# Mictronics/multi-sdr-gps-sim

Hardware: NVIDIA H100
Metric: IQ Msamples/s (higher is better)
Workload: dtype f64 NCO / int32 accumulate / int8 out

## Files before the change

include/gpsb200.h:

```cpp
#ifndef GPSB200_H
#define GPSB200_H

#include <stdbool.h>
#include <stddef.h>
#include <stdint.h>

#ifdef __cplusplus
extern "C" {
#endif

#define GPSB200_SAMPLERATE        3000000
#define GPSB200_BLOCK_SAMPLES     300000
#define GPSB200_BLOCK_ELEMS       600000
#define GPSB200_MAX_CHAN          32
#define GPSB200_NAV_WORDS         60
#define GPSB200_CA_LEN            1023
#define GPSB200_SC08              1
#define GPSB200_SC16              2
#define GPSB200_HACKRF_BUFFER     262144

enum {
    GPSB200_OK = 0,
    GPSB200_ERR_ARG = -1,
    GPSB200_ERR_CUDA = -2,
// ... 55 lines not shown

int gpsb200_synth_blocks_device(gpsb200_ctx_t *ctx, const gpsb200_chan_t *chans, int nblk, int nchan,
                                int sample_size, void *dst_device, void *stream,
                                double *carr_phase_out, gpsb200_stats_t *stats);

typedef struct gpsb200_slice_link {
    int32_t prn_first[GPSB200_MAX_CHAN];
    int32_t prn_last[GPSB200_MAX_CHAN];
    int32_t reset_inside[GPSB200_MAX_CHAN];
    double first_phase[GPSB200_MAX_CHAN];
    double value[GPSB200_MAX_CHAN];
} gpsb200_slice_link_t;
int gpsb200_slice_prepare(gpsb200_ctx_t *ctx, const gpsb200_chan_t *chans, int nblk, int nchan, int sample_size,
                          void *dst_device, void *dst_host, void *stream, gpsb200_slice_link_t *link);
int gpsb200_slice_wait(gpsb200_ctx_t *ctx);
int gpsb200_slice_probe(gpsb200_ctx_t *ctx, const int32_t *prn_in, const double *phase_guess_in, int eager);
int gpsb200_slice_finish(gpsb200_ctx_t *ctx, const int32_t *prn_in, const double *phase_in, int32_t *prn_out,
                         double *phase_out, gpsb200_stats_t *stats);
typedef void (*gpsb200_handoff_fn)(void *user, const int32_t *prn_out, const double *phase_out);
int gpsb200_slice_finish_cb(gpsb200_ctx_t *ctx, const int32_t *prn_in, const double *phase_in, int32_t *prn_out,
                            double *phase_out, gpsb200_stats_t *stats, gpsb200_handoff_fn handoff, void *user);
int gpsb200_slice_link_host(const gpsb200_chan_t *chans, int nblk, int nchan, gpsb200_slice_link_t *link);
int gpsb200_link_apply(const gpsb200_slice_link_t *link, int nchan, const int32_t *prn_in, const double *phase_in,
                       int32_t *prn_out, double *phase_out);

int gpsb200_debug_corrupt_chain(gpsb200_ctx_t *ctx, int on);

int gpsb200_debug_run_checkpoints(gpsb200_ctx_t *ctx, int nblk, int nchan, void *out);

int gpsb200_debug_block_probes(gpsb200_ctx_t *ctx, int nblk, int nchan, void *probes_out, double *seg_out,
                               double *guess_out);

int gpsb200_debug_synth_shape(gpsb200_ctx_t *ctx, int nblk, int nchan, int sample_size, const char **kernel,
                              int *ctas_per_block, int *runs_per_cta);

const char *gpsb200_synth_kernel_name(const gpsb200_ctx_t *ctx, int nchan);

int gpsb200_replay_device(gpsb200_ctx_t *ctx, void *dst_device, void *stream, int kernel_mask);

double gpsb200_carrier_advance(double carr_phase, double f_carr, int64_t nsamples);

int gpsb200_carrier_chain(const gpsb200_chan_t *chans, int nblk, int nchan, const double *phase_in,
                          double *phase_out, int threads);

int gpsb200_carrier_chain_device(gpsb200_ctx_t *ctx, const gpsb200_chan_t *chans, int nblk, int nchan,
                                 const double *phase_in, double *phase_out);

int gpsb200_carrier_probe_fixup(double start, double guess, double f_carr, int64_t nsamples, double *end_out);

int gpsb200_span_chain_host(const double *f_carr, int nblk, double start_true, double start_guess, double *starts_out);

int gpsb200_checkpoint_segments_host(double start_true, double start_guess, double f_carr, int run_samples,
                                     double *starts_out, int *nseg_out);

int gpsb200_carrier_probe_host(double guess, double f_carr, int64_t nsamples, int run_samples, int mode, void *probe_out,
                               double *seg_out);

int gpsb200_lanes_model_block(const gpsb200_chan_t *chans, int nchan, const uint32_t *nav, int run_samples, int force,
                              int16_t *iq, double *carr_out, int64_t *counters, uint32_t *signs);

int gpsb200_lanes_window_band_host(const uint32_t *steps, const uint32_t *bases, int64_t n, uint8_t *out);

int gpsb200_codegen(int prn, uint8_t ca[GPSB200_CA_LEN]);

#define GPSB200_ACQ_MAX_MS    100
#define GPSB200_ACQ_MAX_BINS  1024
#define GPSB200_ACQ_CODE_SAMPLES 3000
typedef struct gpsb200_acq_config {
    int64_t s0;
    int32_t ms;
    int32_t nprn;
    int32_t prn[32];
    double f_lo_hz;
    double step_hz;
    int32_t nbins;
    int32_t reserved;
} gpsb200_acq_config_t;
typedef struct gpsb200_acq_result {
    int32_t prn;
    int32_t bin;
    int32_t delay;
    int32_t reserved;
    double doppler_hz;
    double delay_chips;
    uint64_t p1, p2;
    double ratio;
} gpsb200_acq_result_t;
int gpsb200_acquire(gpsb200_ctx_t *ctx, const void *iq, int64_t nsamples, int sample_size, const gpsb200_acq_config_t *cfg,
                    gpsb200_acq_result_t *res, uint64_t *grid);
int gpsb200_acquire_device(gpsb200_ctx_t *ctx, const void *iq_device, int64_t nsamples, int sample_size,
                           const gpsb200_acq_config_t *cfg, gpsb200_acq_result_t *res, uint64_t *grid, void *stream);
int gpsb200_acquire_windows(gpsb200_ctx_t *ctx, const void *iq, int64_t nsamples, int sample_size,
                            const gpsb200_acq_config_t *cfg, const double *f_lo_prn, gpsb200_acq_result_t *res,
                            uint64_t *grid);
int gpsb200_debug_acq_split(gpsb200_ctx_t *ctx, int force, int nprn, int nbins);
int gpsb200_acquire_windows_device(gpsb200_ctx_t *ctx, const void *iq_device, int64_t nsamples, int sample_size,
                                   const gpsb200_acq_config_t *cfg, const double *f_lo_prn, gpsb200_acq_result_t *res,
                                   uint64_t *grid, void *stream);

#define GPSB200_TRK_CODE_STEP_NOM 1464583848u
#define GPSB200_TRK_CODE_STEP_MIN 1464095816u
#define GPSB200_TRK_CODE_STEP_MAX 1465072205u
#define GPSB200_TRK_FLL_EPOCHS    200
#define GPSB200_TRK_MAX_CHAN      32
typedef struct gpsb200_track_state {
    int32_t prn;
// ... 383 lines not shown
```

multi-sdr-gps-sim_b200/__init__.py:

```python
from .api import (
    BLOCK_ELEMS, BLOCK_SAMPLES, SC08, SC16, Chan, Config, Context, GpsB200Error, Stats,
    bind_numa, carrier_advance, span_chain_host, lanes_model_block, lanes_window_band, link_apply, slice_link_host, SliceLink, carrier_chain, codegen, scenario, lib, lib_path, CHAN_DTYPE,
    ScenarioConfig, LiveScenario, SteerState, parse_steer, KEYS, ERR_END, almanac_read, ALMANAC_RECORD_DTYPE, checkpoint_segments_host, RUN_CKPT_DTYPE,
    carrier_probe_host, CARRIER_PROBE_DTYPE, AcqConfig, ACQ_RESULT_DTYPE, ACQ_CODE_SAMPLES, acq_window_samples,
    TRACK_STATE_DTYPE, TRACK_EPOCH_DTYPE, NAV_BIT_DTYPE, NAV_WORD_DTYPE, NAV_SYNC_DTYPE, track_start, nav_decode, nav_word_check,
    nav_parity, EPHEMERIS_DTYPE, IONO_DTYPE, PVT_CHAN_DTYPE, PVT_CONFIG_DTYPE, FIX_DTYPE, FIX_OK, FIX_FEW,
    FIX_NO_CONVERGENCE, PVT_MAX_ITER, nav_words_of_frame, nav_ephemeris, nav_time_anchor, pvt_config,
    RAIM_CONFIG_DTYPE, RAIM_DTYPE, RAIM_PASS, RAIM_EXCLUDED, RAIM_ALERT, RAIM_UNAVAILABLE, RAIM_MAX_DOF,
    RAIM_MAX_EXCLUDE, raim_config, raim_thresholds, ARAIM_CONFIG_DTYPE, ARAIM_DTYPE, araim_config, araim_kfa,
    COARSE_CONFIG_DTYPE, COARSE_DTYPE, FIX_AMBIGUOUS, coarse_config, rinex_ephemeris,
    SEARCH_CONFIG_DTYPE, SEARCH_DTYPE, SEARCH_NODES, search_config, search_nodes,
    SKY_DTYPE, nav_almanac, almanac_predict,
    SNAPSHOT_CONFIG_DTYPE, SNAPSHOT_DTYPE, SNAP_OK, SNAP_WEAK, SNAP_NO_CONVERGENCE, SNAP_ITERATIONS, SNAP_MAX_ITER,
    snapshot_config,
)
from .synthetic import synthetic_chans
from . import sharding
```

multi-sdr-gps-sim_b200/api.py:

```python
import ctypes as C
import os

import numpy as np

BLOCK_SAMPLES = 300000
BLOCK_ELEMS = 600000
SC08, SC16 = 1, 2

_HERE = os.path.dirname(os.path.abspath(__file__))


def lib_path():
    return os.path.join(_HERE, "libgpsb200.so")


class GpsB200Error(RuntimeError):
    def __init__(self, code, msg):
        super().__init__("gpsb200 error %d: %s" % (code, msg))
        self.code = code


class Chan(C.Structure):
    _fields_ = [("prn", C.c_int32), ("iword", C.c_int32), ("ibit", C.c_int32), ("icode", C.c_int32),
                ("nav_frame", C.c_int32), ("reserved", C.c_int32),
# ... 292 lines not shown
    return rec, int(wna.value)


SKY_DTYPE = np.dtype([("prn", "<i4"), ("valid", "<i4"), ("el_deg", "<f8"), ("az_deg", "<f8"), ("range_m", "<f8"),
                      ("doppler_hz", "<f8")])
assert SKY_DTYPE.itemsize == 40


def almanac_predict(rec, week, sow, x_a):
    r = np.ascontiguousarray(rec, dtype=ALMANAC_RECORD_DTYPE)
    assert r.size == 32
    x = np.ascontiguousarray(x_a, dtype=np.float64).reshape(3)
    out = np.zeros(32, SKY_DTYPE)
    rc = lib().gpsb200_almanac_predict(r.ctypes.data, int(week), float(sow), x.ctypes.data, out.ctypes.data)
    if rc:
        raise GpsB200Error(rc, "gpsb200_almanac_predict")
    return out


def nav_time_anchor(words, sync):
    w = np.ascontiguousarray(words, dtype=NAV_WORD_DTYPE)
    sy = np.array(sync, dtype=NAV_SYNC_DTYPE).reshape(1)
    ep, ms = C.c_int32(0), C.c_int64(0)
    rc = lib().gpsb200_nav_time_anchor(w.ctypes.data if w.size else None, w.size, sy.ctypes.data, C.byref(ep), C.byref(ms))
    if rc:
        raise GpsB200Error(rc, "gpsb200_nav_time_anchor")
    return int(ep.value), int(ms.value)


def pvt_config(s0, step, nfix, iono=None):
    c = np.zeros(1, PVT_CONFIG_DTYPE)[0]
    c["s0"], c["step"], c["nfix"] = int(s0), int(step), int(nfix)
    if iono is not None:
        c["iono"] = 1
        c["alpha"], c["beta"] = np.asarray(iono[0], np.float64), np.asarray(iono[1], np.float64)
    return c


HANDOFF_FN = C.CFUNCTYPE(None, C.c_void_p, C.POINTER(C.c_int32), C.POINTER(C.c_double))

_lib = None

EXPORTS = ["gpsb200_create", "gpsb200_destroy", "gpsb200_last_error", "gpsb200_version", "gpsb200_set_nav",
           "gpsb200_synth_blocks", "gpsb200_synth_blocks_scatter", "gpsb200_synth_blocks_device", "gpsb200_replay_device",
           "gpsb200_carrier_advance", "gpsb200_carrier_chain", "gpsb200_carrier_chain_device", "gpsb200_carrier_probe_fixup",
           "gpsb200_codegen", "gpsb200_acquire", "gpsb200_acquire_device", "gpsb200_acquire_windows",
           "gpsb200_acquire_windows_device", "gpsb200_debug_acq_split", "gpsb200_nav_almanac", "gpsb200_almanac_predict", "gpsb200_track_start",
           "gpsb200_track",
           "gpsb200_track_device", "gpsb200_nav_decode", "gpsb200_nav_word_check", "gpsb200_nav_parity",
           "gpsb200_nav_ephemeris", "gpsb200_nav_time_anchor", "gpsb200_pvt", "gpsb200_pvt_replay",
           "gpsb200_pvt_raim", "gpsb200_raim_thresholds", "gpsb200_pvt_araim", "gpsb200_araim_kfa", "gpsb200_pvt_coarse", "gpsb200_pvt_search", "gpsb200_search_nodes", "gpsb200_snapshot_measure", "gpsb200_snapshot_measure_device", "gpsb200_pvt_snapshot", "gpsb200_pvt_snapshot_search", "gpsb200_rinex_ephemeris", "gpsb200_bind_numa", "gpsb200_span_chain_host", "gpsb200_lanes_model_block",
           "gpsb200_lanes_window_band_host", "gpsb200_slice_prepare", "gpsb200_slice_probe",
           "gpsb200_slice_finish", "gpsb200_slice_finish_cb", "gpsb200_slice_wait", "gpsb200_link_apply", "gpsb200_slice_link_host", "gpsb200_debug_corrupt_chain", "gpsb200_synth_kernel_name",
           "gpsb200_debug_run_checkpoints", "gpsb200_checkpoint_segments_host",
           "gpsb200_carrier_probe_host", "gpsb200_debug_block_probes", "gpsb200_debug_synth_shape",
           "gpsb200_scenario_create", "gpsb200_scenario_destroy", "gpsb200_scenario_error",
           "gpsb200_scenario_blocks", "gpsb200_scenario_channels", "gpsb200_scenario_nav_frames",
           "gpsb200_scenario_chans", "gpsb200_scenario_nav", "gpsb200_scenario_almanac_date", "gpsb200_almanac_read",
           "gpsb200_scenario_open", "gpsb200_scenario_advance", "gpsb200_scenario_frame", "gpsb200_scenario_key",
           "gpsb200_scenario_steer_state", "gpsb200_scenario_open_now", "gpsb200_scenario_create_now",
           "gpsb200_scenario_start_date", "gpsb200_scenario_start_time",
           "fifo_create", "fifo_destroy", "fifo_wait_next", "fifo_wait_full", "fifo_halt", "fifo_acquire",
           "fifo_enqueue", "fifo_dequeue", "fifo_release", "fifo_set_compat_drop",
           "gpsb200_iqfile_start", "gpsb200_iqfile_stop", "gpsb200_fifo_push", "gpsb200_fifo_push_flush"]


def lib():
    global _lib
    if _lib is None:
        if not os.path.exists(lib_path()):
            raise GpsB200Error(-2, "libgpsb200.so not built (run __graft_entry__.build()); there is no CPU fallback")
        L = C.CDLL(lib_path())
        L.gpsb200_create.argtypes = [C.POINTER(Config), C.POINTER(C.c_void_p)]
        L.gpsb200_destroy.argtypes = [C.c_void_p]
        L.gpsb200_last_error.argtypes = [C.c_void_p]
        L.gpsb200_last_error.restype = C.c_char_p
        L.gpsb200_version.restype = C.c_char_p
        L.gpsb200_set_nav.argtypes = [C.c_void_p, C.c_int, C.c_int, C.c_void_p]
        L.gpsb200_synth_blocks.argtypes = [C.c_void_p, C.c_void_p, C.c_int, C.c_int, C.c_int, C.c_void_p,
                                           C.c_void_p, C.POINTER(Stats)]
        L.gpsb200_synth_blocks_scatter.argtypes = [C.c_void_p, C.c_void_p, C.c_int, C.c_int, C.c_int, C.c_void_p,
                                                   C.c_void_p, C.POINTER(Stats)]
        L.gpsb200_synth_blocks_device.argtypes = [C.c_void_p, C.c_void_p, C.c_int, C.c_int, C.c_int, C.c_void_p,
                                                  C.c_void_p, C.c_void_p, C.POINTER(Stats)]
        L.gpsb200_replay_device.argtypes = [C.c_void_p, C.c_void_p, C.c_void_p, C.c_int]
        L.gpsb200_carrier_advance.argtypes = [C.c_double, C.c_double, C.c_int64]
        L.gpsb200_carrier_advance.restype = C.c_double
        L.gpsb200_codegen.argtypes = [C.c_int, C.c_void_p]
        L.gpsb200_scenario_create.argtypes = [C.POINTER(ScenarioConfig), C.POINTER(C.c_void_p)]
        L.gpsb200_scenario_destroy.argtypes = [C.c_void_p]
        L.gpsb200_scenario_error.argtypes = [C.c_void_p]
        L.gpsb200_scenario_error.restype = C.c_char_p
        for fn in ("blocks", "channels", "nav_frames"):
            getattr(L, "gpsb200_scenario_" + fn).argtypes = [C.c_void_p]
        L.gpsb200_scenario_chans.argtypes = [C.c_void_p]
        L.gpsb200_scenario_chans.restype = C.c_void_p
        L.gpsb200_scenario_nav.argtypes = [C.c_void_p]
        L.gpsb200_scenario_nav.restype = C.c_void_p
        L.gpsb200_scenario_almanac_date.argtypes = [C.c_void_p]
        L.gpsb200_scenario_almanac_date.restype = C.c_char_p
        L.gpsb200_almanac_read.argtypes = [C.c_char_p, C.c_void_p, C.POINTER(C.c_int32)]
        L.gpsb200_scenario_open.argtypes = [C.POINTER(ScenarioConfig), C.POINTER(C.c_void_p)]
        L.gpsb200_scenario_open_now.argtypes = [C.POINTER(ScenarioConfig), C.POINTER(C.c_void_p)]
        L.gpsb200_scenario_create_now.argtypes = [C.POINTER(ScenarioConfig), C.POINTER(C.c_void_p)]
        L.gpsb200_scenario_start_date.argtypes = [C.c_void_p]
        L.gpsb200_scenario_start_date.restype = C.c_char_p
        L.gpsb200_scenario_start_time.argtypes = [C.c_void_p, C.POINTER(C.c_int32), C.POINTER(C.c_double)]
        L.gpsb200_scenario_advance.argtypes = [C.c_void_p, C.c_int, C.c_void_p, C.POINTER(C.c_int32)]
        L.gpsb200_scenario_frame.argtypes = [C.c_void_p, C.c_int]
        L.gpsb200_scenario_frame.restype = C.c_void_p
        L.gpsb200_scenario_key.argtypes = [C.c_void_p, C.c_int]
        L.gpsb200_scenario_steer_state.argtypes = [C.c_void_p, C.POINTER(SteerState)]
        L.gpsb200_carrier_probe_fixup.argtypes = [C.c_double, C.c_double, C.c_double, C.c_int64, C.POINTER(C.c_double)]
        L.gpsb200_carrier_chain_device.argtypes = [C.c_void_p, C.c_void_p, C.c_int, C.c_int, C.c_void_p, C.c_void_p]
        L.gpsb200_carrier_chain.argtypes = [C.c_void_p, C.c_int, C.c_int, C.c_void_p, C.c_void_p, C.c_int]
        L.gpsb200_span_chain_host.argtypes = [C.c_void_p, C.c_int, C.c_double, C.c_double, C.c_void_p]
        L.gpsb200_slice_prepare.argtypes = [C.c_void_p, C.c_void_p, C.c_int, C.c_int, C.c_int, C.c_void_p, C.c_void_p,
                                            C.c_void_p, C.POINTER(SliceLink)]
        L.gpsb200_slice_finish_cb.argtypes = [C.c_void_p, C.c_void_p, C.c_void_p, C.c_void_p, C.c_void_p, C.POINTER(Stats),
                                              HANDOFF_FN, C.c_void_p]
        L.gpsb200_slice_wait.argtypes = [C.c_void_p]
        L.gpsb200_slice_link_host.argtypes = [C.c_void_p, C.c_int, C.c_int, C.POINTER(SliceLink)]
        L.gpsb200_slice_probe.argtypes = [C.c_void_p, C.c_void_p, C.c_void_p, C.c_int]
        L.gpsb200_slice_finish.argtypes = [C.c_void_p, C.c_void_p, C.c_void_p, C.c_void_p, C.c_void_p, C.POINTER(Stats)]
        L.gpsb200_link_apply.argtypes = [C.POINTER(SliceLink), C.c_int, C.c_void_p, C.c_void_p, C.c_void_p, C.c_void_p]
        L.gpsb200_debug_corrupt_chain.argtypes = [C.c_void_p, C.c_int]
        L.gpsb200_debug_run_checkpoints.argtypes = [C.c_void_p, C.c_int, C.c_int, C.c_void_p]
        L.gpsb200_checkpoint_segments_host.argtypes = [C.c_double, C.c_double, C.c_double, C.c_int, C.c_void_p,
                                                       C.POINTER(C.c_int)]
        L.gpsb200_carrier_probe_host.argtypes = [C.c_double, C.c_double, C.c_int64, C.c_int, C.c_int, C.c_void_p,
                                                 C.c_void_p]
        L.gpsb200_debug_block_probes.argtypes = [C.c_void_p, C.c_int, C.c_int, C.c_void_p, C.c_void_p, C.c_void_p]
        L.gpsb200_debug_synth_shape.argtypes = [C.c_void_p, C.c_int, C.c_int, C.c_int, C.POINTER(C.c_char_p),
                                                C.POINTER(C.c_int), C.POINTER(C.c_int)]
        L.gpsb200_synth_kernel_name.argtypes = [C.c_void_p, C.c_int]
        L.gpsb200_synth_kernel_name.restype = C.c_char_p
        L.gpsb200_acquire.argtypes = [C.c_void_p, C.c_void_p, C.c_int64, C.c_int, C.POINTER(AcqConfig), C.c_void_p,
                                      C.c_void_p]
        L.gpsb200_acquire_device.argtypes = [C.c_void_p, C.c_void_p, C.c_int64, C.c_int, C.POINTER(AcqConfig),
                                             C.c_void_p, C.c_void_p, C.c_void_p]
        L.gpsb200_acquire_windows.argtypes = [C.c_void_p, C.c_void_p, C.c_int64, C.c_int, C.POINTER(AcqConfig),
                                              C.c_void_p, C.c_void_p, C.c_void_p]
        L.gpsb200_acquire_windows_device.argtypes = [C.c_void_p, C.c_void_p, C.c_int64, C.c_int, C.POINTER(AcqConfig),
                                                     C.c_void_p, C.c_void_p, C.c_void_p, C.c_void_p]
        L.gpsb200_debug_acq_split.argtypes = [C.c_void_p, C.c_int, C.c_int, C.c_int]
        L.gpsb200_nav_almanac.argtypes = [C.c_void_p, C.c_int64, C.c_int32, C.c_void_p, C.POINTER(C.c_int32)]
        L.gpsb200_almanac_predict.argtypes = [C.c_void_p, C.c_int32, C.c_double, C.c_void_p, C.c_void_p]
        L.gpsb200_track_start.argtypes = [C.c_int, C.c_double, C.c_int64, C.c_void_p]
        L.gpsb200_track.argtypes = [C.c_void_p, C.c_void_p, C.c_int64, C.c_int, C.c_int64, C.c_void_p, C.c_int, C.c_int,
                                    C.c_void_p, C.c_void_p]
        L.gpsb200_track_device.argtypes = [C.c_void_p, C.c_void_p, C.c_int64, C.c_int, C.c_int64, C.c_void_p, C.c_int,
                                           C.c_int, C.c_void_p, C.c_void_p, C.c_void_p]
        L.gpsb200_nav_decode.argtypes = [C.c_void_p, C.c_int64, C.c_void_p, C.c_int64, C.c_void_p, C.c_int64, C.c_void_p]
        L.gpsb200_nav_word_check.argtypes = [C.c_uint32, C.c_uint32, C.POINTER(C.c_uint32)]
        L.gpsb200_nav_parity.argtypes = [C.c_uint32, C.c_int, C.c_int]
        L.gpsb200_nav_parity.restype = C.c_uint32
        L.gpsb200_nav_ephemeris.argtypes = [C.c_void_p, C.c_int64, C.c_void_p, C.c_void_p]
        L.gpsb200_nav_time_anchor.argtypes = [C.c_void_p, C.c_int64, C.c_void_p, C.POINTER(C.c_int32),
                                              C.POINTER(C.c_int64)]
        L.gpsb200_pvt.argtypes = [C.c_void_p, C.c_void_p, C.c_int, C.c_void_p, C.c_void_p, C.c_int, C.c_void_p, C.c_void_p,
                                  C.c_void_p]
        L.gpsb200_pvt_replay.argtypes = [C.c_void_p, C.c_void_p]
        L.gpsb200_pvt_raim.argtypes = [C.c_void_p, C.c_void_p, C.c_int, C.c_void_p, C.c_void_p, C.c_int, C.c_void_p,
                                       C.c_void_p, C.c_void_p, C.c_void_p, C.c_void_p]
        L.gpsb200_raim_thresholds.argtypes = [C.c_double, C.c_double, C.c_void_p, C.c_void_p]
        L.gpsb200_pvt_araim.argtypes = L.gpsb200_pvt_raim.argtypes
        L.gpsb200_araim_kfa.argtypes = [C.c_double, C.c_double, C.c_void_p, C.c_void_p]
        L.gpsb200_pvt_coarse.argtypes = L.gpsb200_pvt_raim.argtypes + [C.c_void_p]
        L.gpsb200_pvt_search.argtypes = L.gpsb200_pvt_coarse.argtypes + [C.c_void_p]
        L.gpsb200_search_nodes.argtypes = [C.c_int, C.c_void_p]
        L.gpsb200_snapshot_measure.argtypes = [C.c_void_p, C.c_void_p, C.c_int64, C.c_int, C.POINTER(AcqConfig),
                                               C.c_void_p, C.c_void_p, C.c_void_p]
        L.gpsb200_snapshot_measure_device.argtypes = L.gpsb200_snapshot_measure.argtypes + [C.c_void_p]
        L.gpsb200_pvt_snapshot.argtypes = [C.c_void_p, C.c_void_p, C.c_int, C.c_void_p, C.c_void_p, C.c_void_p,
                                           C.c_void_p, C.c_void_p, C.c_void_p, C.c_void_p]
        L.gpsb200_pvt_snapshot_search.argtypes = L.gpsb200_pvt_snapshot.argtypes + [C.c_void_p]
        L.gpsb200_rinex_ephemeris.argtypes = [C.c_char_p, C.c_int, C.c_int32, C.c_double, C.c_void_p]
        _lib = L
    return _lib


def bind_numa(device=0):
# ... 26 lines not shown
        raise GpsB200Error(rc, "gpsb200_carrier_chain")
    return out


def lanes_model_block(chans_row, nav_frame, run_samples=2400, force=0, want_signs=False):
    a = np.ascontiguousarray(chans_row, dtype=CHAN_DTYPE)
    nv = np.ascontiguousarray(nav_frame, dtype=np.uint32)
    iq = np.zeros(BLOCK_ELEMS, np.int16)
    co = np.zeros(a.size, np.float64)
    cnt = np.zeros(4, np.int64)
    signs = np.zeros((a.size, BLOCK_SAMPLES // 96, 3), np.uint32) if want_signs else None
    L = lib()
    L.gpsb200_lanes_model_block.argtypes = [C.c_void_p, C.c_int, C.c_void_p, C.c_int, C.c_int, C.c_void_p, C.c_void_p, C.c_void_p,
                                            C.c_void_p]
    rc = L.gpsb200_lanes_model_block(a.ctypes.data, a.size, nv.ctypes.data, run_samples, force, iq.ctypes.data, co.ctypes.data,
                                     cnt.ctypes.data, None if signs is None else signs.ctypes.data)
    if rc:
        raise GpsB200Error(rc, "gpsb200_lanes_model_block")
    return (iq, co, cnt, signs) if want_signs else (iq, co, cnt)


def lanes_window_band(steps, bases):
    st, bs = np.broadcast_arrays(np.asarray(steps, np.uint32), np.asarray(bases, np.uint32))
    st = np.ascontiguousarray(st.ravel())
    bs = np.ascontiguousarray(bs.ravel())
    out = np.zeros(st.size, np.uint8)
    L = lib()
    L.gpsb200_lanes_window_band_host.argtypes = [C.c_void_p, C.c_void_p, C.c_int64, C.c_void_p]
    rc = L.gpsb200_lanes_window_band_host(st.ctypes.data, bs.ctypes.data, st.size, out.ctypes.data)
    if rc:
        raise GpsB200Error(rc, "gpsb200_lanes_window_band_host")
    return out.astype(bool)


def span_chain_host(f_carr, start_true, start_guess):
    f = np.ascontiguousarray(f_carr, dtype=np.float64)
    out = np.zeros(f.size + 1)
    rc = lib().gpsb200_span_chain_host(f.ctypes.data, f.size, float(start_true), float(start_guess), out.ctypes.data)
    if rc < 0:
        raise GpsB200Error(rc, "gpsb200_span_chain_host")
    return out if rc == 1 else None


def checkpoint_segments_host(start_true, start_guess, f_carr, run_samples=2400):
    out = np.zeros(8)
    nseg = C.c_int(0)
    rc = lib().gpsb200_checkpoint_segments_host(float(start_true), float(start_guess), float(f_carr), int(run_samples),
                                            out.ctypes.data, C.byref(nseg))
    if rc < 0:
        raise GpsB200Error(rc, "gpsb200_checkpoint_segments_host")
    return rc == 1, out[:nseg.value]


def carrier_probe_host(guess, f_carr, nsamples=BLOCK_SAMPLES, run_samples=2400, mode=1):
    probe = np.zeros(1, CARRIER_PROBE_DTYPE)
    seg = np.zeros((2, 7))
    rc = lib().gpsb200_carrier_probe_host(float(guess), float(f_carr), int(nsamples), int(run_samples), int(mode),
                                          probe.ctypes.data, seg.ctypes.data)
    if rc:
        raise GpsB200Error(rc, "gpsb200_carrier_probe_host")
    return probe[0], seg


def slice_link_host(chans):
    a = np.ascontiguousarray(chans, dtype=CHAN_DTYPE)
    link = SliceLink()
    rc = lib().gpsb200_slice_link_host(a.ctypes.data, a.shape[0], a.shape[1], C.byref(link))
    if rc:
        raise GpsB200Error(rc, "gpsb200_slice_link_host")
    return link


def link_apply(link, nchan, prn_in=None, phase_in=None):
    pi = None if prn_in is None else np.ascontiguousarray(prn_in, dtype=np.int32)
    xi = None if phase_in is None else np.ascontiguousarray(phase_in, dtype=np.float64)
    po, xo = np.zeros(nchan, np.int32), np.zeros(nchan, np.float64)
    rc = lib().gpsb200_link_apply(C.byref(link), nchan, None if pi is None else pi.ctypes.data,
                                  None if xi is None else xi.ctypes.data, po.ctypes.data, xo.ctypes.data)
    if rc:
        raise GpsB200Error(rc, "gpsb200_link_apply")
    return po, xo


def almanac_read(path):
    rec = np.zeros(32, ALMANAC_RECORD_DTYPE)
    valid = C.c_int32(0)
    rc = lib().gpsb200_almanac_read(os.fsencode(path), rec.ctypes.data, C.byref(valid))
    if rc:
        raise GpsB200Error(rc, "cannot open almanac file %s" % path)
    return bool(valid.value), rec


def _scenario_config(nav_file, lat, lon, height, seconds, max_chan=12, motion_file=None, start=None,
                     ionosphere=True, pluto_gain=False, rinex3=False, target=None, almanac_file=None, interactive=False):
    cfg = ScenarioConfig()
    cfg.nav_file = os.fsencode(nav_file)
    cfg.motion_file = os.fsencode(motion_file) if motion_file else None
    cfg.lat_deg, cfg.lon_deg, cfg.height_m = lat, lon, height
    cfg.duration_ds = int(seconds * 10.0 + 0.5)
    cfg.max_chan = max_chan
    cfg.ionosphere_enable = 1 if ionosphere else 0
    cfg.pluto_gain = 1 if pluto_gain else 0
    cfg.rinex3 = 1 if rinex3 else 0
    cfg.almanac_file = os.fsencode(almanac_file) if almanac_file else None
    cfg.interactive = 1 if interactive else 0
    if target is not None:
# ... 478 lines not shown
```

multi-sdr-gps-sim_b200/csrc/gpsb200_api.cu:

```cuda
#include <cuda_runtime.h>
#include <sched.h>

#include <algorithm>
#include <atomic>
#include <chrono>
#include <condition_variable>
#include <functional>
#include <mutex>
#include <cctype>
#include <cmath>
#include <cstdio>
#include <cstring>
#include <memory>
#include <string>
#include <thread>
#include <vector>

#include "../../include/gpsb200.h"
#include "acquire.h"
#include "snapshot.h"
#include "device_buffer.h"
#include "track.h"
#include "pvt.h"
#include "nco_exact.h"
// ... 665 lines not shown
    CU(cudaEventRecord(ctx->ev[kEvCallEnd], call.stream));
    CU(cudaMemcpyAsync(ctx->h_chain_errors, ctx->d_chain_errors, sizeof(int), cudaMemcpyDeviceToHost, sp));
    ctx->last = call_args(ctx, call, 0, call.nblk);
    ctx->have_last = true;
    return GPSB200_OK;
}

int call_verdict(gpsb200_ctx *ctx, const Call &call) {
    int bad = *ctx->h_chain_errors;
    for (int i = 0; i < call.rows; i++)
        for (int c = 0; c < call.nchan; c++) {
            const double want = ctx->seg_expect[(size_t) i * call.nchan + c];
            if (want >= 0.0 && f64_bits(want) != f64_bits(ctx->h_seg_end[(size_t) i * call.nchan + c])) ++bad;
        }
    if (bad != 0)
        return fail(ctx, GPSB200_ERR_INTERNAL, "carrier chain self-check failed on " + std::to_string(bad) + " blocks");
    return GPSB200_OK;
}

void seed_chain(std::vector<ChainState> &chain, int nchan, const int32_t *prn_in, const double *phase_in) {
    for (int c = 0; c < nchan; c++) {
        chain[c].prn = (prn_in && phase_in && prn_in[c] > 0) ? prn_in[c] : 0;
        chain[c].phase = chain[c].prn ? phase_in[c] : 0.0;
    }
}

void export_chain(const std::vector<ChainState> &chain, int nchan, int32_t *prn_out, double *phase_out) {
    for (int c = 0; c < nchan; c++) {
        if (prn_out) prn_out[c] = chain[c].prn;
        if (phase_out) phase_out[c] = chain[c].prn > 0 ? chain[c].phase : 0.0;
    }
}

int small_call(gpsb200_ctx *ctx, Call &call, double *carr_phase_out, gpsb200_stats_t *stats) {
    const int nblk = call.nblk, nchan = call.nchan;
    cudaStream_t s = call.stream;
    double t0 = now_ms();
    int rc = prepare_blocks(ctx, call.chans, 0, nblk, nchan, call.chain);
    if (rc) return rc;
    const int nruns = ctx->nruns, run = ctx->cfg.run_samples;
    ctx->pool->run(nchan, [&](int c_lo, int c_hi) {
        for (int c = c_lo; c < c_hi; c++) {
            ChainState stc = call.chain[c];
            for (int b = 0; b < nblk; b++) {
                const BlockChanDev &p = ctx->h_bc[(size_t) b * nchan + c];
                RunCkpt *ck = ctx->h_ck + (size_t) b * nruns * nchan + c;
                if (p.prn <= 0) {
                    stc.prn = 0;
                    for (int r = 0; r < nruns; r++) ck[(size_t) r * nchan] = RunCkpt{0.0, 0.0, 0u, 0u};
                    continue;
                }
                if (stc.prn != p.prn) stc.phase = p.carr_in;
                stc.prn = p.prn;
                double x = stc.phase, y = p.code0;
                int iword = p.nav0 & 0xFF, ibit = (p.nav0 >> 8) & 0xFF, icode = (p.nav0 >> 16) & 0xFF;
                const WalkConst wx = walk_const(p.c_carr), wy = walk_const(p.c_code);
                for (int r = 0; r < nruns; r++) {
                    ck[(size_t) r * nchan] = RunCkpt{x, y, (uint32_t) iword | ((uint32_t) ibit << 8) | ((uint32_t) icode << 16), 0u};
                    int64_t periods = 0, dummy = 0;
                    nco_advance<NCO_CARRIER>(x, wx, run, dummy);
                    nco_advance<NCO_CODE>(y, wy, run, periods);
                    nav_advance(iword, ibit, icode, periods);
                }
                stc.phase = x;
            }
            call.chain[c] = stc;
        }
    });
    call.st.host_chain_ms = now_ms() - t0;
    rc = upload_nav(ctx, s);
    if (rc) return rc;
    const size_t cnt = (size_t) nblk * nchan;
    CU(cudaEventRecord(ctx->ev[kEvCallStart], s));
    CU(cudaMemcpyAsync(ctx->d_bc, ctx->h_bc, cnt * sizeof(BlockChanDev), cudaMemcpyHostToDevice, s));
    CU(cudaMemcpyAsync(ctx->d_ck, ctx->h_ck, cnt * nruns * sizeof(RunCkpt), cudaMemcpyHostToDevice, s));
    const SynthArgs a = call_args(ctx, call, 0, nblk);
    CU(launch_tables(a, s));
    CU(launch_synth(a, s));
    CU(cudaEventRecord(ctx->ev[kEvCallEnd], s));
    call.st.launches = 2;
    call.st.h2d_bytes = (int64_t) (cnt * (sizeof(BlockChanDev) + nruns * sizeof(RunCkpt)));
    if (call.host()) {
        rc = download(ctx, call, 0, nblk, s);
        if (rc) return rc;
        CU(cudaStreamSynchronize(s));
    }
    ctx->have_last = false;
    export_chain(call.chain, nchan, nullptr, carr_phase_out);
    if (stats) *stats = call.st;
    return GPSB200_OK;
}

int run_pipeline(gpsb200_ctx *ctx, Call &call, double *carr_phase_out, gpsb200_stats_t *stats) {
    ctx->trace_t0 = now_ms();
    trace(ctx, "call");
    if (call.nblk <= kHostChainBlocks && !ctx->fault_inject_chain) return small_call(ctx, call, carr_phase_out, stats);
    cudaStream_t sp = ctx->s_pre;
    int rc = call_open(ctx, call);
    if (rc) return rc;
    const auto &segs = call.segs;
    const int nseg = (int) segs.size();
    if (!call.host()) {
        std::vector<ChainState> guess = call.chain;
        for (int i = 0; i < nseg; i++) {
            cudaStream_t sw = (i & 1) ? ctx->s_ck : sp;
            rc = seg_params(ctx, call, segs[i].first, segs[i].second, sw, &guess, nullptr);
            if (rc) return rc;
            rc = seg_probe(ctx, call, segs[i].first, segs[i].second, sw);
            if (rc) return rc;
            CU(cudaEventRecord(ctx->ev_seg[i], sw));
        }
        trace(ctx, "speculative work enqueued");
        for (int i = 0; i < nseg; i++) {
            rc = seg_scan(ctx, call, i, ctx->ev_seg[i], nullptr);
            if (rc) return rc;
        }
        CU(cudaStreamSynchronize(ctx->s_ck));
// ... 291 lines not shown
const char *gpsb200_last_error(const gpsb200_ctx_t *ctx) { return ctx ? ctx->err.c_str() : "null context"; }

int gpsb200_codegen(int prn, uint8_t ca[GPSB200_CA_LEN]) { return ca_code(prn, ca) == 0 ? GPSB200_OK : GPSB200_ERR_ARG; }

double gpsb200_carrier_advance(double carr_phase, double f_carr, int64_t nsamples) {
    const double c = f_carr * (1.0 / (double) GPSB200_SAMPLERATE);
    int64_t dummy = 0;
    nco_advance<NCO_CARRIER>(carr_phase, c, nsamples, dummy);
    return carr_phase;
}

int gpsb200_carrier_probe_fixup(double start, double guess, double f_carr, int64_t nsamples, double *end_out) {
    const double c = f_carr * (1.0 / (double) GPSB200_SAMPLERATE);
    CarrierProbe p;
    carrier_probe(guess, c, nsamples, p);
    double xe = 0.0;
    const bool ok = carrier_fixup(start, c, p, xe);
    if (ok && end_out) *end_out = xe;
    return ok ? 1 : 0;
}

int gpsb200_span_chain_host(const double *f_carr, int nblk, double start_true, double start_guess, double *starts_out) {
    if (!f_carr || nblk < 1 || !starts_out) return GPSB200_ERR_ARG;
    const double delt = 1.0 / (double) GPSB200_SAMPLERATE;
    std::vector<CarrierProbe> probes(nblk);
    std::vector<double> cc(nblk);
    std::vector<SpanBlockState> spec(nblk);
    uint64_t acc = phase_to_fix(start_guess);
    const double guess0 = fix_to_phase(acc);
    for (int j = 0; j < nblk; j++) {
        cc[j] = f_carr[j] * delt;
        carrier_probe(fix_to_phase(acc), cc[j], GPSB200_BLOCK_SAMPLES, probes[j]);
        acc = guess_block(acc, cc[j]);
    }
    CarrierProbe sum{}, part{};
    bool ok[2];
    for (int V = 0; V < 2; V++) {
        span_chain(probes.data(), OneSatellite{cc.data()}, nblk, 1, guess0, V, part, ok[V], spec.data());
        if (V == 0) {
            sum.x_w = part.x_w;
            sum.n_w = part.n_w;
        }
        sum.x_end[V] = part.x_end[V];
        sum.m_pos[V] = ok[V] ? part.m_pos[V] : 0.0;
        sum.m_neg[V] = ok[V] ? part.m_neg[V] : 0.0;
    }
    double xe, d;
    int v;
    if (!carrier_fixup(start_true, cc[0], sum, xe, &v, &d, 1.0)) return 0;
    starts_out[0] = start_true;
    for (int j = 1; j < nblk; j++) starts_out[j] = spec[j].start[v] + d;
    starts_out[nblk] = xe;
    return 1;
}

int gpsb200_checkpoint_segments_host(double start_true, double start_guess, double f_carr, int run_samples,
                                     double *starts_out, int *nseg_out) {
    if (!starts_out || run_samples <= 0 || GPSB200_BLOCK_SAMPLES % run_samples != 0) return GPSB200_ERR_ARG;
    const double c = f_carr * (1.0 / (double) GPSB200_SAMPLERATE);
    const int nruns = GPSB200_BLOCK_SAMPLES / run_samples, nseg = ckpt_segments(nruns);
    CarrierProbe p;
    double seg[kSegStates];
    carrier_probe_walk2(start_guess, c, GPSB200_BLOCK_SAMPLES, p, seg, nruns, run_samples);
    if (nseg_out) *nseg_out = nseg;
    starts_out[0] = start_true;
    for (int j = 1; j < kCkptSegs; j++) starts_out[j] = NAN;
    double xe, d;
    int v;
    if (!carrier_fixup(start_true, c, p, xe, &v, &d)) return 0;
    for (int j = first_derived_segment(p, nseg, nruns, run_samples); j < nseg; j++)
        starts_out[j] = seg[v * (kCkptSegs - 1) + j - 1] + d;
    return 1;
}

int gpsb200_carrier_probe_host(double guess, double f_carr, int64_t nsamples, int run_samples, int mode, void *probe_out,
                               double *seg_out) {
    if (!probe_out || nsamples < 0 || nsamples >= ((int64_t) 1 << 31) || (mode != 0 && mode != 1) || run_samples < 0 ||
        (run_samples > 0 && nsamples % run_samples != 0))
        return GPSB200_ERR_ARG;
    const double c = f_carr * (1.0 / (double) GPSB200_SAMPLERATE);
    const int nruns = run_samples > 0 ? (int) (nsamples / run_samples) : 0;
    double *seg = run_samples > 0 ? seg_out : nullptr;
    if (seg)
        for (int k = 0; k < kSegStates; k++) seg[k] = NAN;
    CarrierProbe p{};
    if (mode == 0) {
        for (int v = 0; v < 2; v++)
            carrier_probe_walk(guess, c, nsamples, v, p.n_w, p.x_w, p.x_end[v], p.m_pos[v], p.m_neg[v],
                               seg ? seg + v * (kCkptSegs - 1) : nullptr, nruns, run_samples);
    } else {
        carrier_probe_walk2(guess, c, nsamples, p, seg, nruns, run_samples);
    }
    memcpy(probe_out, &p, sizeof p);
    return GPSB200_OK;
}

int gpsb200_carrier_chain(const gpsb200_chan_t *chans, int nblk, int nchan, const double *phase_in,
                          double *phase_out, int threads) {
    if (!chans || !phase_out || nblk < 0 || nchan < 1) return GPSB200_ERR_ARG;
    const double delt = 1.0 / (double) GPSB200_SAMPLERATE;
    auto work = [&](int lo, int hi) {
        for (int c = lo; c < hi; c++) {
            int prn = 0;
            double ph = phase_in ? phase_in[c] : 0.0;
            for (int b = 0; b < nblk; b++) {
                const gpsb200_chan_t &in = chans[(size_t) b * nchan + c];
// ... 567 lines not shown
```

multi-sdr-gps-sim_b200/csrc/nco_exact.h:

```cpp
#pragma once
#include <stdint.h>
#include <string.h>

#if defined(__CUDACC__)
#define GPSB_HD __host__ __device__ __forceinline__
#else
#define GPSB_HD inline
#endif

namespace gpsb200 {

enum NcoKind { NCO_CODE = 0, NCO_CARRIER = 1 };

constexpr double kBelowOne = 0.99999999999999988897769753748434595763683319091796875;

GPSB_HD uint64_t f64_bits(double v) {
#if defined(__CUDA_ARCH__)
    return (uint64_t) __double_as_longlong(v);
#else
    uint64_t b;
    memcpy(&b, &v, 8);
    return b;
#endif
}
// ... 445 lines not shown
    const bool neg = c0 < 0.0;
    double x = p0.x_end[V];
    double mp = 0.5 * p0.m_pos[V], mn = 0.5 * p0.m_neg[V];
    if (!(mp > 0.0 && mn > 0.0)) return;
    for (int j = 1; j < nblk_span; j++) {
        const size_t i = (size_t) j * stride;
        blocks[i].start[V] = x;
        double c;
        int32_t prn;
        param(j, c, prn);
        if (prn != prn0 || c == 0.0 || (c < 0.0) != neg) return;
        int v;
        double d, xe, pmp, pmn;
        if (!carrier_fixup(x, c, probes[i], xe, &v, &d, 0.5, &pmp, &pmn)) return;
        const double a = 0.5 * probes[i].m_pos[v] - d, b = 0.5 * probes[i].m_neg[v] + d;
        if (a < mp) mp = a;
        if (b < mn) mn = b;
        if (0.5 * pmp < mp) mp = 0.5 * pmp;
        if (0.5 * pmn < mn) mn = 0.5 * pmn;
        x = xe;
    }
    sum.n_w = p0.n_w;
    sum.x_w = p0.x_w;
    sum.x_end[V] = x;
    sum.m_pos[V] = mp;
    sum.m_neg[V] = mn;
    ok = true;
}

inline double carrier_drift_per_step(double c) {
    if (c == 0.0) return 0.0;
    const uint64_t cb = f64_bits(c) & 0x7FFFFFFFFFFFFFFFull;
    const int ec = (int) (cb >> 52);
    if (ec == 0 || ec >= 1022) return 0.0;
    const double ac = bits_f64(cb);
    double tot = 0.0;
    for (int ex = ec + 1; ex <= 1022; ex++) {
        if (ex - ec >= 54) break;
        const double lo = bits_f64((uint64_t) ex << 52);
        const double stepd = (lo + ac) - lo;
        tot += (stepd - ac) * lo;
    }
    return c > 0.0 ? tot : -tot;
}

GPSB_HD void nav_advance(int &iword, int &ibit, int &icode, int64_t periods) {
    int64_t t = (int64_t) icode + periods;
    icode = (int) (t % 20);
    t = (int64_t) ibit + t / 20;
    ibit = (int) (t % 30);
    iword += (int) (t / 30);
}

}
```

Baseline: 70970.

## Replace per-run code NCO advance with periodic stretch-jump code walk

Host-side checkpoint generation now computes the code-phase NCO checkpoints with a new code_walk_runs routine. It walks one code period segment by segment, then jumps over repeated periods using floating-point rounding margins, instead of calling nco_advance for every run. The carrier walk is split into its own loop. This targets host CPU cost of preparing run checkpoints per channel. It adds complex exactness logic with a fallback path, plus a new host test entry point.

```diff
diff --git a/include/gpsb200.h b/include/gpsb200.h
--- a/include/gpsb200.h
+++ b/include/gpsb200.h
@@ -131,6 +131,9 @@
 
 int gpsb200_checkpoint_segments_host(double start_true, double start_guess, double f_carr, int run_samples,
                                      double *starts_out, int *nseg_out);
+
+int gpsb200_code_walk_host(double code0, double c_code, int run_samples, int method, double *y_out,
+                           int64_t *periods_out, int32_t *stats_out);
 
 int gpsb200_carrier_probe_host(double guess, double f_carr, int64_t nsamples, int run_samples, int mode, void *probe_out,
                                double *seg_out);
diff --git a/multi-sdr-gps-sim_b200/__init__.py b/multi-sdr-gps-sim_b200/__init__.py
--- a/multi-sdr-gps-sim_b200/__init__.py
+++ b/multi-sdr-gps-sim_b200/__init__.py
@@ -2,7 +2,7 @@
     BLOCK_ELEMS, BLOCK_SAMPLES, SC08, SC16, Chan, Config, Context, GpsB200Error, Stats,
     bind_numa, carrier_advance, span_chain_host, lanes_model_block, lanes_window_band, link_apply, slice_link_host, SliceLink, carrier_chain, codegen, scenario, lib, lib_path, CHAN_DTYPE,
     ScenarioConfig, LiveScenario, SteerState, parse_steer, KEYS, ERR_END, almanac_read, ALMANAC_RECORD_DTYPE, checkpoint_segments_host, RUN_CKPT_DTYPE,
-    carrier_probe_host, CARRIER_PROBE_DTYPE, AcqConfig, ACQ_RESULT_DTYPE, ACQ_CODE_SAMPLES, acq_window_samples,
+    carrier_probe_host, code_walk_host, CARRIER_PROBE_DTYPE, AcqConfig, ACQ_RESULT_DTYPE, ACQ_CODE_SAMPLES, acq_window_samples,
     TRACK_STATE_DTYPE, TRACK_EPOCH_DTYPE, NAV_BIT_DTYPE, NAV_WORD_DTYPE, NAV_SYNC_DTYPE, track_start, nav_decode, nav_word_check,
     nav_parity, EPHEMERIS_DTYPE, IONO_DTYPE, PVT_CHAN_DTYPE, PVT_CONFIG_DTYPE, FIX_DTYPE, FIX_OK, FIX_FEW,
     FIX_NO_CONVERGENCE, PVT_MAX_ITER, nav_words_of_frame, nav_ephemeris, nav_time_anchor, pvt_config,
diff --git a/multi-sdr-gps-sim_b200/api.py b/multi-sdr-gps-sim_b200/api.py
--- a/multi-sdr-gps-sim_b200/api.py
+++ b/multi-sdr-gps-sim_b200/api.py
@@ -368,7 +368,7 @@
            "gpsb200_pvt_raim", "gpsb200_raim_thresholds", "gpsb200_pvt_araim", "gpsb200_araim_kfa", "gpsb200_pvt_coarse", "gpsb200_pvt_search", "gpsb200_search_nodes", "gpsb200_snapshot_measure", "gpsb200_snapshot_measure_device", "gpsb200_pvt_snapshot", "gpsb200_pvt_snapshot_search", "gpsb200_rinex_ephemeris", "gpsb200_bind_numa", "gpsb200_span_chain_host", "gpsb200_lanes_model_block",
            "gpsb200_lanes_window_band_host", "gpsb200_slice_prepare", "gpsb200_slice_probe",
            "gpsb200_slice_finish", "gpsb200_slice_finish_cb", "gpsb200_slice_wait", "gpsb200_link_apply", "gpsb200_slice_link_host", "gpsb200_debug_corrupt_chain", "gpsb200_synth_kernel_name",
-           "gpsb200_debug_run_checkpoints", "gpsb200_checkpoint_segments_host",
+           "gpsb200_debug_run_checkpoints", "gpsb200_checkpoint_segments_host", "gpsb200_code_walk_host",
            "gpsb200_carrier_probe_host", "gpsb200_debug_block_probes", "gpsb200_debug_synth_shape",
            "gpsb200_scenario_create", "gpsb200_scenario_destroy", "gpsb200_scenario_error",
            "gpsb200_scenario_blocks", "gpsb200_scenario_channels", "gpsb200_scenario_nav_frames",
@@ -444,6 +444,8 @@
         L.gpsb200_debug_run_checkpoints.argtypes = [C.c_void_p, C.c_int, C.c_int, C.c_void_p]
         L.gpsb200_checkpoint_segments_host.argtypes = [C.c_double, C.c_double, C.c_double, C.c_int, C.c_void_p,
                                                        C.POINTER(C.c_int)]
+        L.gpsb200_code_walk_host.argtypes = [C.c_double, C.c_double, C.c_int, C.c_int, C.c_void_p, C.c_void_p,
+                                             C.c_void_p]
         L.gpsb200_carrier_probe_host.argtypes = [C.c_double, C.c_double, C.c_int64, C.c_int, C.c_int, C.c_void_p,
                                                  C.c_void_p]
         L.gpsb200_debug_block_probes.argtypes = [C.c_void_p, C.c_int, C.c_int, C.c_void_p, C.c_void_p, C.c_void_p]
@@ -576,6 +578,16 @@
     return rc == 1, out[:nseg.value]
 
 
+def code_walk_host(code0, c_code, run_samples=2400, method=0):
+    n = BLOCK_SAMPLES // int(run_samples)
+    y, periods, stats = np.zeros(n), np.zeros(n, np.int64), np.zeros(4, np.int32)
+    rc = lib().gpsb200_code_walk_host(float(code0), float(c_code), int(run_samples), int(method), y.ctypes.data,
+                                      periods.ctypes.data, stats.ctypes.data)
+    if rc < 0:
+        raise GpsB200Error(rc, "gpsb200_code_walk_host")
+    return y, periods, stats
+
+
 def carrier_probe_host(guess, f_carr, nsamples=BLOCK_SAMPLES, run_samples=2400, mode=1):
     probe = np.zeros(1, CARRIER_PROBE_DTYPE)
     seg = np.zeros((2, 7))
diff --git a/multi-sdr-gps-sim_b200/csrc/gpsb200_api.cu b/multi-sdr-gps-sim_b200/csrc/gpsb200_api.cu
--- a/multi-sdr-gps-sim_b200/csrc/gpsb200_api.cu
+++ b/multi-sdr-gps-sim_b200/csrc/gpsb200_api.cu
@@ -741,17 +741,24 @@
                 }
                 if (stc.prn != p.prn) stc.phase = p.carr_in;
                 stc.prn = p.prn;
-                double x = stc.phase, y = p.code0;
-                int iword = p.nav0 & 0xFF, ibit = (p.nav0 >> 8) & 0xFF, icode = (p.nav0 >> 16) & 0xFF;
-                const WalkConst wx = walk_const(p.c_carr), wy = walk_const(p.c_code);
+                double x = stc.phase;
+                const WalkConst wx = walk_const(p.c_carr);
                 for (int r = 0; r < nruns; r++) {
-                    ck[(size_t) r * nchan] = RunCkpt{x, y, (uint32_t) iword | ((uint32_t) ibit << 8) | ((uint32_t) icode << 16), 0u};
-                    int64_t periods = 0, dummy = 0;
+                    ck[(size_t) r * nchan].x = x;
+                    int64_t dummy = 0;
                     nco_advance<NCO_CARRIER>(x, wx, run, dummy);
-                    nco_advance<NCO_CODE>(y, wy, run, periods);
-                    nav_advance(iword, ibit, icode, periods);
                 }
                 stc.phase = x;
+                int iword = p.nav0 & 0xFF, ibit = (p.nav0 >> 8) & 0xFF, icode = (p.nav0 >> 16) & 0xFF;
+                int64_t done = 0;
+                code_walk_runs(p.code0, walk_const(p.c_code), nruns, run, [&](int r, double y, int64_t P) {
+                    nav_advance(iword, ibit, icode, P - done);
+                    done = P;
+                    RunCkpt &o = ck[(size_t) r * nchan];
+                    o.y = y;
+                    o.nav = (uint32_t) iword | ((uint32_t) ibit << 8) | ((uint32_t) icode << 16);
+                    o.pad = 0u;
+                });
             }
             call.chain[c] = stc;
         }
@@ -1149,6 +1156,38 @@
     for (int j = 1; j < nblk; j++) starts_out[j] = spec[j].start[v] + d;
     starts_out[nblk] = xe;
     return 1;
+}
+
+int gpsb200_code_walk_host(double code0, double c_code, int run_samples, int method, double *y_out,
+                           int64_t *periods_out, int32_t *stats_out) {
+    if (!y_out || !periods_out || run_samples <= 0 || GPSB200_BLOCK_SAMPLES % run_samples != 0 || method < 0 ||
+        method > 2)
+        return GPSB200_ERR_ARG;
+    const int nruns = GPSB200_BLOCK_SAMPLES / run_samples;
+    if (method == 0) {
+        CodeWalkStats st;
+        code_walk_runs(code0, walk_const(c_code), nruns, run_samples, [&](int r, double y, int64_t P) {
+            y_out[r] = y;
+            periods_out[r] = P;
+        }, &st);
+        if (stats_out) {
+            stats_out[0] = st.walked;
+            stats_out[1] = st.jumped;
+            stats_out[2] = st.fallback;
+            stats_out[3] = st.iters;
+        }
+        return GPSB200_OK;
+    }
+    double y = code0;
+    int64_t P = 0;
+    for (int r = 0; r < nruns; r++) {
+        y_out[r] = y;
+        periods_out[r] = P;
+        if (method == 1) nco_advance_generic<NCO_CODE>(y, c_code, run_samples, P);
+        else
+            for (int i = 0; i < run_samples; i++) nco_step<NCO_CODE>(y, c_code, P);
+    }
+    return GPSB200_OK;
 }
 
 int gpsb200_checkpoint_segments_host(double start_true, double start_guess, double f_carr, int run_samples,
diff --git a/multi-sdr-gps-sim_b200/csrc/nco_exact.h b/multi-sdr-gps-sim_b200/csrc/nco_exact.h
--- a/multi-sdr-gps-sim_b200/csrc/nco_exact.h
+++ b/multi-sdr-gps-sim_b200/csrc/nco_exact.h
@@ -521,4 +521,161 @@
     iword += (int) (t / 30);
 }
 
-}
+constexpr int kCodeSegs = 32;
+
+GPSB_HD void code_margins(double y, double &m_up, double &m_dn) {
+    const uint64_t b = f64_bits(y);
+    const int ex = (int) (b >> 52);
+    const double lo = bits_f64((uint64_t) ex << 52), u = bits_f64((uint64_t) (ex - 52) << 52);
+    double up = (lo + lo - (u + u)) - y, dn = y - (lo + u);
+    if (ex == 1023 + 9) {
+        if (y < 1023.0) {
+            const double t = (1023.0 - u) - y;
+            if (t < up) up = t;
+        } else {
+            const double t = y - 1023.0;
+            if (t < dn) dn = t;
+        }
+    }
+    if (up < m_up) m_up = up;
+    if (dn < m_dn) m_dn = dn;
+}
+
+struct CodeStretch {
+    int32_t seg_t[kCodeSegs];
+    double seg_x[kCodeSegs];
+    int nseg;
+    int32_t L;
+    double end;
+    double m_up, m_dn;
+};
+
+GPSB_HD void code_stretch_begin(CodeStretch &s, double x, int32_t n, double &nd) {
+    s.seg_t[0] = 0;
+    s.seg_x[0] = x;
+    s.nseg = 0;
+    s.L = 0;
+    s.end = x;
+    s.m_up = s.m_dn = 1024.0;
+    nd = (double) n;
+}
+
+GPSB_HD bool code_stretch_step(CodeStretch &s, const WalkConst &w, int32_t n, double &nd) {
+    if (s.nseg == kCodeSegs) return false;
+    double x = s.end;
+    const bool rounded = s.nseg > 0;
+    s.seg_t[s.nseg] = n - (int32_t) nd;
+    s.seg_x[s.nseg] = x;
+    s.nseg++;
+    if (rounded) code_margins(x, s.m_up, s.m_dn);
+    double aj;
+    int64_t p = 0;
+    const bool wr = walk_iteration<NCO_CODE>(x, w, nd, p, &aj);
+    if (rounded || aj != s.end) code_margins(aj, s.m_up, s.m_dn);
+    if (wr) {
+        code_margins(x + 1023.0, s.m_up, s.m_dn);
+        s.L = n - (int32_t) nd;
+    }
+    s.end = x;
+    return true;
+}
+
+GPSB_HD double code_stretch_at(const CodeStretch &s, const WalkConst &w, int32_t j) {
+    int i = 0;
+#pragma unroll
+    for (int h = kCodeSegs / 2; h > 0; h >>= 1)
+        if (i + h < s.nseg && s.seg_t[i + h] <= j) i += h;
+    const double x = s.seg_x[i];
+    const int ex = (int) ((f64_bits(x) >> 52) & 0x7FF);
+    const double lo = bits_f64((uint64_t) ex << 52);
+    const double stepd = ex == w.ec ? w.ac : (lo + w.ac) - lo;
+    return x + (double) (j - s.seg_t[i]) * stepd;
+}
+
+GPSB_HD int32_t code_jumps(const CodeStretch &s, double delta, bool tie_c) {
+    if (delta == 0.0) return 1 << 30;
+    if (tie_c && (((long long) (delta * 0x1p43)) & 1)) return 0;
+    const double ad = delta > 0.0 ? delta : -delta;
+    const double room = delta > 0.0 ? s.m_up : s.m_dn, back = delta > 0.0 ? s.m_dn : s.m_up;
+    if (!(back >= 0.0) || !(room >= ad)) return 0;
+    const double q = room / ad;
+    double nn = floor_nonneg(q < 0x1p30 ? q : 0x1p30);
+    while (nn * ad > room) nn -= 1.0;
+    return (int32_t) nn;
+}
+
+GPSB_HD bool code_jumps_apply(const WalkConst &w) { return w.fast && !w.neg && w.ec < 1023; }
+
+struct CodeWalkStats {
+    int walked;
+    int jumped;
+    int fallback;
+    int iters;
+};
+
+template <class Rec>
+GPSB_HD void code_walk_runs(double y, const WalkConst &w, int nruns, int run_samples, Rec rec,
+                            CodeWalkStats *st = nullptr) {
+    if (st) *st = CodeWalkStats{0, 0, 0, 0};
+    if (nruns <= 0) return;
+    int r = 0;
+    int32_t t = 0;
+    int64_t P = 0;
+    if (w.c != 0.0 && code_jumps_apply(w)) {
+        const double c44 = w.ac * 0x1p44;
+        const bool tie_c = c44 == floor_nonneg(c44);
+        const int32_t last = (nruns - 1) * run_samples;
+        bool post = false;
+        bool walking = true;
+        CodeStretch s;
+        double nd, delta = 0.0;
+        int32_t N = 0, n = 0;
+        code_stretch_begin(s, y, last, nd);
+        while (r < nruns) {
+            if (walking) {
+                if (nd > 0.0 && s.L == 0) {
+                    if (!code_stretch_step(s, w, last - t, nd)) break;
+                    if (st) st->iters++;
+                }
+                if (nd == 0.0 || s.L > 0) {
+                    delta = s.end - y;
+                    N = post && s.L > 0 ? code_jumps(s, delta, tie_c) : 0;
+                    walking = false;
+                    if (st) st->walked++;
+                }
+            } else {
+                const int32_t o = r * run_samples - t;
+                const int32_t m = s.L > 0 ? o / s.L : 0;
+                if (m <= N) {
+                    rec(r, code_stretch_at(s, w, o - m * s.L) + (double) m * delta, P + m);
+                    r++;
+                    n = m;
+                } else {
+                    if (st) st->jumped += N;
+                    y = s.end + (double) N * delta;
+                    t += (N + 1) * s.L;
+                    P += N + 1;
+                    post = true;
+                    walking = true;
+                    n = 0;
+                    code_stretch_begin(s, y, last - t, nd);
+                }
+            }
+        }
+        if (r == nruns) {
+            if (st) st->jumped += n;
+            return;
+        }
+    }
+    if (st) st->fallback = 1;
+    for (; r < nruns; r++) {
+        int64_t p = 0;
+        const int it = nco_advance<NCO_CODE>(y, w, (int64_t) r * run_samples - t, p);
+        if (st) st->iters += it;
+        t = r * run_samples;
+        P += p;
+        rec(r, y, P);
+    }
+}
+
+}
```

Result: no change. 70990, median of 6 (+0.0%).
